# ishine/TargetDiarization

Measured on AMD Instinct MI355X. Metric: real-time factor (audio-sec/wall-sec) full infer() pipe, 16kHz mono, 1/2/4/8 GPU, higher is better.
Workload: dtype f32 (split-f16 x3: fp32-accurate products from three f16 MFMA passes, fp32 accumulate); 1 GPU; BASELINE configs[3]: 1800 s synthetic conversation (two alternating speakers, 20 % overlap) = 180 x 10 s windows: MossFormer2 (90 windows per launch) -> loudness swap -> ERes2NetV2 on every 10 s window of both streams + cosine vs a target embedding -> Paraformer (SANM encoder, CIF predictor, NAR decoder, argmax tokens + timestamps) on 30 s segments of both streams -> CT-Transformer punctuation of ; windows_per_launch=90

## Files before the change

targetdiarization_amd/csrc/eres2net.hip:

```cpp
#include <hip/hip_runtime.h>

#include <algorithm>
#include <cmath>
#include <string>
#include <vector>

#include "../../include/tdx.h"
#include "epilogues.hpp"
#include "weight_pack.hpp"
#include "weight_planes.hpp"

using namespace tdx;

namespace {

constexpr int NSTAGE = 4, SCALE = 4, EMB = 192;
const int kBlocks[NSTAGE] = {3, 4, 6, 3};
const int kPlanes[NSTAGE] = {64, 128, 256, 512};
const int kStride[NSTAGE] = {1, 2, 2, 2};

__global__ __launch_bounds__(256) void stem_kernel(const float* __restrict__ feat, const float* __restrict__ w9,
                                                    const float* __restrict__ bias, float* __restrict__ out, int F, long rows) {
    const long i = (long)blockIdx.x * 256 + threadIdx.x;
    if (i >= rows * 16) return;
// ... 73 lines not shown
struct EpiAffGate {
    const float* b; const float* x; long ldx; const float* y; long ldy; float* out; long ldo; int C;
    __device__ float col(int, int n) const { return b[n]; }
    __device__ EpiNone row(int, int) const { return EpiNone{}; }
    __device__ float2 aux(int, int m, int n, EpiNone) const {
        return n < C ? make_float2(x[(long)m * (int)ldx + n], y[(long)m * (int)ldy + n]) : make_float2(0.f, 0.f);
    }
    __device__ void store(int, int m, int n, float v, EpiNone, float c, float2 xy) const {
        if (n >= C) return;
        const float att = 1.0f + tanhf(v + c);
        out[(long)m * (int)ldo + n] = xy.x * att + xy.y * (2.0f - att);
    }
};


struct ChainX3Args {
    const float* in; long ldin;
    const unsigned char* wp; const float* ws; int wk;
    int cinp;
    const float* b;
    float* cat; long ldcat; int coff;
    const float* o1; long ldo1; int next_off; float* spin; int ldspin;
    int H, W;
};
template <int CIN, int TH>
struct ChainX3Cfg {
    static constexpr int KS = (CIN + 15) / 16, CP = KS * 16, PPB = CP * 4 + 16, NT = (CIN + 31) / 32, NB = NT * 32, MT = TH / 4;
    static constexpr int PATCH = (TH + 2) * 34 * PPB, BT = NB * PPB, LDS = PATCH + 2 * BT;
    static constexpr int BQ = NB * (CP / 8) * 2;
    static constexpr int BPT = (BQ + 255) / 256;
};
template <int CIN, int TH>
__global__ __launch_bounds__(256) void chain_conv_x3_kernel(ChainX3Args a) {
    using C = ChainX3Cfg<CIN, TH>;
    constexpr int KS = C::KS, CP = C::CP, PPB = C::PPB, NT = C::NT, MT = C::MT;
    static_assert(PPB % 32 == 16 && TH % 4 == 0 && CIN % 4 == 0, "pitch = odd multiple of 16 B");
    extern __shared__ __attribute__((aligned(16))) unsigned char lds[];
    unsigned char* const patch = lds;
    unsigned char* const bt = lds + C::PATCH;
    const int tid = threadIdx.x, lane = tid & 63, wave = tid >> 6, l31 = lane & 31, h = lane >> 5;
    const int x0 = blockIdx.x * 32, y0 = blockIdx.y * TH, b = blockIdx.z;
    typedef _Float16 h4 __attribute__((ext_vector_type(4)));
    typedef unsigned u32x4 __attribute__((ext_vector_type(4)));
    u32x4 breg[3][C::BPT];
#define TDX_CHAIN_BLOAD(tap_)                                                                                          \
    _Pragma("unroll") for (int i = 0; i < C::BPT; ++i) {                                                               \
// ... 95 lines not shown
    TDX_CHAIN_BSTORE(4) TDX_CHAIN_BLOAD(7) TDX_CHAIN_TAP(3) __syncthreads();
    TDX_CHAIN_BSTORE(5) TDX_CHAIN_BLOAD(8) TDX_CHAIN_TAP(4) __syncthreads();
    TDX_CHAIN_BSTORE(6) TDX_CHAIN_TAP(5) __syncthreads();
    TDX_CHAIN_BSTORE(7) TDX_CHAIN_TAP(6) __syncthreads();
    TDX_CHAIN_BSTORE(8) TDX_CHAIN_TAP(7) __syncthreads();
    TDX_CHAIN_TAP(8)
#undef TDX_CHAIN_TAP
#undef TDX_CHAIN_BSTORE
#undef TDX_CHAIN_BLOAD
#pragma unroll
    for (int n = 0; n < NT; ++n) {
        const int c = n * 32 + l31;
        const bool real = c < CIN;
#pragma unroll
        for (int m = 0; m < MT; ++m) {
            const int y = y0 + MT * wave + m;
            if (y >= a.H) continue;
#pragma unroll
            for (int i = 0; i < 16; ++i) {
                const int x = x0 + (i & 3) + 8 * (i >> 2) + 4 * h;
                if (x >= a.W) continue;
                const long mrow = ((long)b * a.H + y) * a.W + x;
                const float sp = relu20(acc[m][n][i] * sc[n] + bias[n]);
                if (real) a.cat[mrow * a.ldcat + a.coff + c] = sp;
                if (a.spin && c < a.ldspin) a.spin[mrow * a.ldspin + c] = real ? sp + nx[n][m][i] : 0.f;
            }
        }
    }
}
template <int CIN, int TH>
int launch_chain_x3(const ChainX3Args& a, int B, hipStream_t st) {
    using C = ChainX3Cfg<CIN, TH>;
    static const hipError_t attr_rc = hipFuncSetAttribute((const void*)chain_conv_x3_kernel<CIN, TH>, hipFuncAttributeMaxDynamicSharedMemorySize, C::LDS);
    if (attr_rc != hipSuccess) return tdx::fail_hip(attr_rc, __FILE__, __LINE__);
    hipLaunchKernelGGL((chain_conv_x3_kernel<CIN, TH>), dim3((a.W + 31) / 32, (a.H + TH - 1) / TH, B), dim3(256), C::LDS, st, a);
    LAUNCH_CHECK();
    return TDX_OK;
}

struct AffArgs {
    const float* x; long ldx; const float* y; long ldy;
    const float* w0; int ld0; const float* b0;
    const float* w3; int ld3; const float* b3;
    float* out; long ldo; long M;
};
template <int C>
struct AffCfg {
    static constexpr int IP = (C / 4 + 31) / 32 * 32, NT1 = IP / 32, NT2 = C / 32, NCH = 2 * C / 32;
    static constexpr int PA = 36, PT = IP + 4;
    static constexpr int AS = 128 * PA, WS = IP * PA;
    static constexpr int TS = 128 * PT;
    static constexpr int REG1 = (2 * AS > TS ? 2 * AS : TS);
    static constexpr int LDS = (REG1 + 2 * WS + C * PT) * 4;
    static constexpr int WPT = (IP * 8 + 255) / 256;
};
template <int C>
__global__ __launch_bounds__(256, C == 96 ? 2 : 1) void aff_fused_kernel(AffArgs a) {
    using F = AffCfg<C>;
    constexpr int IP = F::IP, NT1 = F::NT1, NT2 = F::NT2, NCH = F::NCH, PA = F::PA, PT = F::PT;
    extern __shared__ __attribute__((aligned(16))) float ldsf[];
    float* const As = ldsf;
    float* const Ws = ldsf + F::REG1;
    float* const W3s = Ws + 2 * F::WS;
    float* const Ts = ldsf;
    const int tid = threadIdx.x, lane = tid & 63, wave = tid >> 6, l31 = lane & 31, h = lane >> 5;
    const long m0 = (long)blockIdx.x * 128;
    f32x4 ra[4], rw[F::WPT];
// ... 78 lines not shown
                const f32x4 bv = *reinterpret_cast<const f32x4*>(Wb + n * 32 * PT + 8 * kk);
#pragma unroll
                for (int j = 0; j < 4; ++j) acc2[n] = __builtin_amdgcn_mfma_f32_32x32x2f32(av[j], bv[j], acc2[n], 0, 0, 0);
            }
        }
    }
#pragma unroll
    for (int n = 0; n < NT2; ++n) {
        const int c = n * 32 + l31;
        const float b3 = a.b3[c];
        float xv[16], yv[16];
#pragma unroll
        for (int r = 0; r < 16; ++r) {
            const long m = min(m0 + wave * 32 + (r & 3) + 8 * (r >> 2) + 4 * h, a.M - 1);
            xv[r] = a.x[m * a.ldx + c]; yv[r] = a.y[m * a.ldy + c];
        }
#pragma unroll
        for (int r = 0; r < 16; ++r) { tdx::touch(xv[r]); tdx::touch(yv[r]); }
#pragma unroll
        for (int r = 0; r < 16; ++r) {
            const long m = m0 + wave * 32 + (r & 3) + 8 * (r >> 2) + 4 * h;
            if (m >= a.M) continue;
            const float att = 1.0f + tanhf(acc2[n][r] + b3);
            a.out[m * a.ldo + c] = xv[r] * att + yv[r] * (2.0f - att);
        }
    }
}
template <int C>
int launch_aff_fused(const AffArgs& a, hipStream_t st) {
    using F = AffCfg<C>;
    static const hipError_t attr_rc = hipFuncSetAttribute((const void*)aff_fused_kernel<C>, hipFuncAttributeMaxDynamicSharedMemorySize, F::LDS);
    if (attr_rc != hipSuccess) return tdx::fail_hip(attr_rc, __FILE__, __LINE__);
    hipLaunchKernelGGL((aff_fused_kernel<C>), dim3((unsigned)((a.M + 127) / 128)), dim3(256), F::LDS, st, a);
    LAUNCH_CHECK();
    return TDX_OK;
}

__global__ __launch_bounds__(256) void split_rows_static_s2_kernel(const float* __restrict__ x, int ld, unsigned char* __restrict__ planes,
                                                                  long R, int K, int Hin, int Win, int Ho, int Wo, float s) {
    const long i = (long)blockIdx.x * 256 + threadIdx.x;
    const int per = K / 8;
    if (i >= R * per) return;
    const long row = i / per;
    const int ch = (int)(i - row * per);
    const long b = row / ((long)Ho * Wo);
    const int r = (int)(row - b * Ho * Wo), ho = r / Wo, wo = r - ho * Wo;
    const float* src = x + ((b * Hin + 2 * ho) * Win + 2 * wo) * ld + ch * 8;
// ... 47 lines not shown
    g.cv_Hin = Hin; g.cv_Win = Win; g.cv_Hout = Hout; g.cv_Wout = Wout; g.cv_stride = stride; g.cv_ntaps = tpb; g.cv_cin = cw.cinp;
    g.cv_taps_total = cw.taps;
    g.zero_row = zero_row;
    if (launch_gemm_h3x<false, false, false, false, EpiStoreZ, 0, true>(g, DS_SPLIT, EpiStoreZ{slab, (long)cw.Npad, M * cw.Npad}, st) != hipSuccess)
        return tdx::fail_hip(hipGetLastError(), __FILE__, __LINE__);
    const long MN = M * cw.Npad;
    hipLaunchKernelGGL(slab_reduce_kernel, dim3((unsigned)((MN / 4 + 255) / 256)), dim3(256), 0, st, slab, DS_SPLIT, MN, cw.Npad, bias, out);
    LAUNCH_CHECK();
    return TDX_OK;
}

}

struct tdx_eres2net {
    int device = 0;
    tdx::DevBuf dev; std::vector<BlockW> blocks; size_t stem_w, stem_b, seg_w, seg_b; ConvW ds; AffW fuse34;
    tdx::DevBuf dev_planes;
    size_t consts = 0;
};

namespace {

int run_aff(const tdx_eres2net* h, const AffW& a, const float* x, long ldx, const float* y, long ldy, float* tbuf, float* out, long ldo,
            long M, hipStream_t st) {
    if (a.C == 96 || a.C == 192) {
        AffArgs fa{x, ldx, y, ldy, h->dev + a.c0.w, a.c0.cinp, h->dev + a.c0.b, h->dev + a.c3.w, a.c3.cinp, h->dev + a.c3.b, out, ldo, M};
        return a.C == 96 ? launch_aff_fused<96>(fa, st) : launch_aff_fused<192>(fa, st);
    }
    {
        GemmSeg s0 = make_seg(x, ldx, h->dev + a.c0.w, 2L * a.C, a.C);
        GemmSeg s1 = make_seg(y, ldy, h->dev + a.c0.w + a.C, 2L * a.C, a.C);
        GemmArgs g = make_args((int)M, a.c0.Npad, s0);
        g.seg[1] = s1; g.nseg = 2;
        if (launch_gemm<false, false, false, false>(g, 1, EpiBiasActN<ActSilu>{h->dev + a.c0.b, tbuf, a.ipad, a.ipad}, st) != hipSuccess)
            return tdx::fail_hip(hipGetLastError(), __FILE__, __LINE__);
    }
    return linear_f32(tbuf, a.ipad, h->dev + a.c3.w, (int)M, a.c3.Npad, a.ipad, EpiAffGate{h->dev + a.c3.b, x, ldx, y, ldy, out, ldo, a.C}, st);
}

int run_aff34_x3(const tdx_eres2net* h, const AffW& a, const float* x, const float* y, float* tbuf, float* out, long M,
                 unsigned char* xP, unsigned char* yP, float* ys, unsigned char* tP, float* ts, const float* inv20, hipStream_t st) {
    const int C = a.C, IP = a.ipad;
    if (tdx::launch_h3_split_rows_static(x, C, xP, M, C, 1024.0f, st) != hipSuccess) return tdx::fail_hip(hipGetLastError(), __FILE__, __LINE__);
    if (tdx::launch_h3_split_rows(y, C, yP, ys, M, C, st) != hipSuccess) return tdx::fail_hip(hipGetLastError(), __FILE__, __LINE__);
    {
        H3Args g{};
        g.seg[0] = h3_seg(xP, inv20, 4L * C, a.c0.hp, a.c0.hs, 4L * 2 * C, C);
        g.seg[0].sa_mul = 0;
        g.seg[1] = h3_seg(yP, ys, 4L * C, a.c0.hp + 4L * C, a.c0.hs, 4L * 2 * C, C);
        g.nseg = 2; g.M = (int)M; g.N = a.c0.Npad;
        if (launch_gemm_h3x<false, false, false, true>(g, 1, EpiBiasActN<ActSilu>{h->dev + a.c0.b, tbuf, IP, IP}, st) != hipSuccess)
            return tdx::fail_hip(hipGetLastError(), __FILE__, __LINE__);
    }
    if (tdx::launch_h3_split_rows(tbuf, IP, tP, ts, M, IP, st) != hipSuccess) return tdx::fail_hip(hipGetLastError(), __FILE__, __LINE__);
    H3Args g{};
    g.seg[0] = h3_seg(tP, ts, 4L * IP, a.c3.hp, a.c3.hs, 4L * IP, IP);
    g.nseg = 1; g.M = (int)M; g.N = a.c3.Npad;
    if (launch_gemm_h3<false>(g, 1, EpiAffGate{h->dev + a.c3.b, x, (long)C, y, (long)C, out, (long)C, C}, st) != hipSuccess)
        return tdx::fail_hip(hipGetLastError(), __FILE__, __LINE__);
    return TDX_OK;
}

struct Dims { int H[5], W[5]; };
inline Dims make_dims(int F) {
    Dims d; d.H[0] = 80; d.W[0] = F;
    for (int s = 0; s < NSTAGE; ++s) {
        d.H[s + 1] = kStride[s] == 1 ? d.H[s] : (d.H[s] - 1) / 2 + 1;
        d.W[s + 1] = kStride[s] == 1 ? d.W[s] : (d.W[s] - 1) / 2 + 1;
    }
    return d;
}

}

extern "C" {

int tdx_eres2net_create(const void* blob, size_t blob_bytes, int device, tdx_eres2net** out) {
    if (!blob || !out) return tdx::fail(TDX_E_INVALID, "tdx_eres2net_create: null argument");
    tdx::Loader ld;
    if (!ld.parse(blob, blob_bytes)) return tdx::fail(TDX_E_BLOB, "tdx_eres2net_create: malformed TDXW blob");
    auto fold = [&](const std::string& wname, const std::string& bname, const std::string& bn, int N, int cin, int taps) -> ConvW {
        const float* W = ld.get(wname, (size_t)N * cin * taps);
        const float* cb = bname.empty() ? nullptr : ld.get(bname, N);
        const float *g = nullptr, *be = nullptr, *mu = nullptr, *var = nullptr;
// ... 131 lines not shown
    if (guard.err != hipSuccess) return tdx::fail_hip(guard.err, __FILE__, __LINE__);
    hipStream_t st = (hipStream_t)stream;
    const Dims d = make_dims(F);
    const size_t rows1 = (size_t)B * 80 * F;
    float* ws = (float*)ws_;
    float* P[3] = {ws, ws + wp.P, ws + 2 * wp.P};
    float* keep3 = ws + 3 * wp.P;
    float* o1 = keep3 + wp.keep3; float* cat = o1 + wp.o1;
    float* spin[2] = {cat + wp.o1, cat + wp.o1 + wp.spin};
    float* tbuf = spin[1] + wp.spin; float* stats = tbuf + wp.tbuf;
    unsigned char* hx = (unsigned char*)(stats + wp.stats);
    unsigned char* hcat = hx + wp.hx * sizeof(float);
    unsigned char* hin = hcat + wp.hcat * sizeof(float);
    float* slab = reinterpret_cast<float*>(hin + wp.hin * sizeof(float));
    const float* inv20 = h->dev + h->consts;
    const float* inv40 = h->dev + h->consts + 1;
    const unsigned char* zero_row = (const unsigned char*)(h->dev + h->consts + 64);

    hipLaunchKernelGGL(stem_kernel, dim3((unsigned)((rows1 * 16 + 255) / 256)), dim3(256), 0, st, feat, h->dev + h->stem_w, h->dev + h->stem_b, P[0], F, (long)rows1);
    LAUNCH_CHECK();
    const float* x = P[0];
    int cur = 0;
    int s = 0, cnt = 0;
    for (const BlockW& b : h->blocks) {
        const int Hin = (cnt == 0) ? d.H[s] : d.H[s + 1], Win = (cnt == 0) ? d.W[s] : d.W[s + 1];
        const int Ho = d.H[s + 1], Wo = d.W[s + 1];
        const long M = (long)B * Ho * Wo;
        const bool last_of_stage3 = (s == 2) && (cnt == kBlocks[2] - 1);
        const int iy = cur < 0 ? 0 : (cur + 1) % 3, ir = cur < 0 ? 1 : (cur + 2) % 3;
        float* y = last_of_stage3 ? keep3 : P[iy];
        float* res = P[ir];
        const bool x3 = b.conv1.hp != nullptr;
        const float* resid = x;
        if (x3) {
            int Hc = Hin, Wc = Win, sc_ = b.stride;
            if (b.stride == 2 && b.cin % 16 == 0) {
                const long R = (long)B * Ho * Wo;
                hipLaunchKernelGGL(split_rows_static_s2_kernel, dim3((unsigned)((R * (b.cin / 8) + 255) / 256)), dim3(256), 0, st,
                                   x, b.cin, hx, R, b.cin, Hin, Win, Ho, Wo, 1024.0f);
                LAUNCH_CHECK();
                Hc = Ho; Wc = Wo; sc_ = 1;
            } else if (tdx::launch_h3_split_rows_static(x, b.cin, hx, (long)B * Hin * Win, b.cin, 1024.0f, st) != hipSuccess)
                return tdx::fail_hip(hipGetLastError(), __FILE__, __LINE__);
            TRY(conv_gemm_h3(hx, inv20, zero_row, b.conv1, B, Hc, Wc, Ho, Wo, sc_, EpiBiasActN<ActRelu20>{h->dev + b.conv1.b, o1, b.w4, b.w4}, st));
            if (b.has_sc) {
                TRY(conv_gemm_h3(hx, inv20, zero_row, b.sc, B, Hc, Wc, Ho, Wo, sc_, EpiBiasActN<>{h->dev + b.sc.b, res, b.cout, b.cout}, st));
                resid = res;
            }
        } else {
            TRY(conv_gemm(x, b.cin, h->dev, b.conv1, B, Hin, Win, Ho, Wo, b.stride, EpiBiasActN<ActRelu20>{h->dev + b.conv1.b, o1, b.w4, b.w4}, st));
            if (b.has_sc) {
                TRY(conv_gemm(x, b.cin, h->dev, b.sc, B, Hin, Win, Ho, Wo, b.stride, EpiBiasActN<>{h->dev + b.sc.b, res, b.cout, b.cout}, st));
                resid = res;
            }
        }
        for (int j = 0; j < SCALE; ++j) {
            const float* in = j == 0 ? o1 : spin[j & 1];
            const long ldin = j == 0 ? b.w4 : b.wpad;
            const bool plain_next = (j + 1 < SCALE) && !b.is_aff;
            EpiChain e{h->dev + b.convs[j].b, cat, b.w4, j * b.width, b.width, b.wpad, o1, b.w4, (j + 1) * b.width,
                       plain_next ? spin[(j + 1) & 1] : nullptr};
            if (b.convs[j].hp && !b.is_aff && (b.width == 24 || b.width == 48)) {
                ChainX3Args ca{in, ldin, b.convs[j].hp, b.convs[j].hs, 9 * b.convs[j].cinp, b.convs[j].cinp, h->dev + b.convs[j].b, cat, b.w4, j * b.width,
                               o1, b.w4, (j + 1) * b.width, plain_next ? spin[(j + 1) & 1] : nullptr, b.wpad, Ho, Wo};
                if (b.width == 24) TRY((launch_chain_x3<24, 4>(ca, B, st)));
                else TRY((launch_chain_x3<48, 4>(ca, B, st)));
            } else if (x3) {
                if (tdx::launch_h3_split_rows_static(in, ldin, hin, M, b.wpad, 512.0f, st) != hipSuccess)
                    return tdx::fail_hip(hipGetLastError(), __FILE__, __LINE__);
                TRY(conv_gemm_h3(hin, inv40, zero_row, b.convs[j], B, Ho, Wo, Ho, Wo, 1, e, st));
            } else {
                TRY(conv_gemm(in, ldin, h->dev, b.convs[j], B, Ho, Wo, Ho, Wo, 1, e, st));
            }
            if (b.is_aff && j + 1 < SCALE)
                TRY(run_aff(h, b.aff[j], cat + j * b.width, b.w4, o1 + (j + 1) * b.width, b.w4, tbuf, spin[(j + 1) & 1], b.wpad, M, st));
        }
        if (x3) {
            if (tdx::launch_h3_split_rows_static(cat, b.w4, hcat, M, b.w4, 1024.0f, st) != hipSuccess)
                return tdx::fail_hip(hipGetLastError(), __FILE__, __LINE__);
            TRY(conv_gemm_h3(hcat, inv20, zero_row, b.conv3, B, Ho, Wo, Ho, Wo, 1, EpiBiasRes<ActRelu20>{h->dev + b.conv3.b, resid, y, b.cout}, st));
        } else {
            TRY(linear_f32(cat, b.w4, h->dev + b.conv3.w, (int)M, b.conv3.Npad, b.conv3.cinp, EpiBiasRes<ActRelu20>{h->dev + b.conv3.b, resid, y, b.cout}, st));
        }
        x = y;
        cur = last_of_stage3 ? -1 : iy;
        if (++cnt == kBlocks[s]) { cnt = 0; ++s; }
    }
    const int i_ds = (cur + 1) % 3, i_fu = (cur + 2) % 3;
    const long M4 = (long)B * d.H[4] * d.W[4];
    if (tdx::launch_h3_split_rows_static(keep3, 1024, hx, (long)B * d.H[3] * d.W[3], 1024, 1024.0f, st) != hipSuccess)
        return tdx::fail_hip(hipGetLastError(), __FILE__, __LINE__);
    if (wp.slab && h->ds.taps == 9 && h->ds.Npad == 2048)
        TRY(conv_gemm_h3_tapsplit(hx, inv20, zero_row, h->ds, B, d.H[3], d.W[3], d.H[4], d.W[4], 2, slab, nullptr, P[i_ds], st));
    else
        TRY(conv_gemm_h3(hx, inv20, zero_row, h->ds, B, d.H[3], d.W[3], d.H[4], d.W[4], 2, EpiBiasActN<>{nullptr, P[i_ds], 2048, 2048}, st));
    const char* aff34_env = getenv("TDX_ERES_AFF34_ROWS");
    const long aff34_min = aff34_env ? atol(aff34_env) : 8192;
    if (M4 >= aff34_min && 2 * M4 <= (long)B * 40960 && h->fuse34.c0.hp && h->fuse34.ipad == 512)
        TRY(run_aff34_x3(h, h->fuse34, x, P[i_ds], tbuf, P[i_fu], M4, hx, hcat, stats, hin, stats + M4, inv20, st));
    else
        TRY(run_aff(h, h->fuse34, x, 2048, P[i_ds], 2048, tbuf, P[i_fu], 2048, M4, st));
    hipLaunchKernelGGL(tstp_kernel, dim3(d.H[4], B), dim3(256), 0, st, P[i_fu], stats, d.W[4], 2048, d.H[4]);
    LAUNCH_CHECK();
    hipLaunchKernelGGL(seg_kernel, dim3(EMB, B), dim3(256), 0, st, stats, h->dev + h->seg_w, h->dev + h->seg_b, emb, 40960);
// ... 6 lines not shown
```

targetdiarization_amd/csrc/gemm_h3.hpp:

```cpp
#pragma once
#include <cstdio>
#include <cstdlib>
#include <typeinfo>
#include <vector>
#include <hip/hip_runtime.h>
#include <stdint.h>

#include "devutil.hpp"
#include "gemm.hpp"

namespace tdx {

typedef _Float16 f16x8 __attribute__((ext_vector_type(8)));

constexpr int H3_BM = 256, H3_BN = 256, H3_BK = 16, H3_THREADS = 512;
constexpr int H3_ROWB = 64;
constexpr int H3_OPER = 256 * H3_ROWB;
constexpr int H3_STAGE = 2 * H3_OPER;
constexpr int H3_NBUF = 4;
constexpr int H3_AUX_AHEAD = 3;
constexpr int H3_LDS = H3_NBUF * H3_STAGE;
constexpr int H3_LDS_EXTRA = 12288;

struct H3Seg {
// ... 221 lines not shown
    h4 a, b;
#pragma unroll
    for (int j = 0; j < 4; ++j) { const _Float16 t = (_Float16)xs[j]; a[j] = t; b[j] = (_Float16)(xs[j] - (float)t); }
    H3Pair r;
    r.hi = __builtin_bit_cast(uint2, a); r.lo = __builtin_bit_cast(uint2, b);
    return r;
}
__device__ __forceinline__ uint4 h3_pair16(int q, float4 v, float s) {
    const H3Pair o = h3_split4(v, s);
    const bool odd = q & 1;
    const uint2 send = odd ? o.hi : o.lo;
    uint2 recv;
    recv.x = (unsigned)__builtin_amdgcn_mov_dpp((int)send.x, 0xB1, 0xF, 0xF, true);
    recv.y = (unsigned)__builtin_amdgcn_mov_dpp((int)send.y, 0xB1, 0xF, 0xF, true);
    return odd ? make_uint4(recv.x, recv.y, o.lo.x, o.lo.y) : make_uint4(o.hi.x, o.hi.y, recv.x, recv.y);
}
__device__ __forceinline__ void h3_emit4(unsigned char* prow, int q, float4 v, float s) {
    *reinterpret_cast<uint4*>(prow + (q >> 1) * 32 + ((q & 1) ? 16 : 0)) = h3_pair16(q, v, s);
}
__device__ __forceinline__ void h3_emit4_pred(unsigned char* prow, int q, float4 v, float s, bool ok) {
    const uint4 w = h3_pair16(q, v, s);
    if (ok) *reinterpret_cast<uint4*>(prow + (q >> 1) * 32 + ((q & 1) ? 16 : 0)) = w;
}
__device__ __forceinline__ float h3_absmax4(float4 v) { return fmaxf(fmaxf(fabsf(v.x), fabsf(v.y)), fmaxf(fabsf(v.z), fabsf(v.w))); }


struct H3PlOut { unsigned char* planes; long pitch; float* scale; float* ss; long seg_stride; };
template <class E, class = void> struct epi_has_plout { static constexpr bool value = false; };
template <class E> struct epi_has_plout<E, decltype((void)&E::plout, void())> { static constexpr bool value = true; };
template <class E, class = void> struct epi_has_rowout { static constexpr bool value = false; };
template <class E> struct epi_has_rowout<E, decltype((void)&E::rowout, void())> { static constexpr bool value = true; };
struct H3Conv {
    const float* w; int wld;
    int ncols;
    unsigned char* planes; long pitch;
    float sv;
    float* u32; int u0; long ld32;
    int S, Sp;
};
template <class E, class = void> struct epi_has_conv { static constexpr bool value = false; };
template <class E> struct epi_has_conv<E, decltype((void)&E::conv, void())> { static constexpr bool value = true; };
constexpr int H3_CONV_STEP = 240, H3_CONV_HALO = 8;
template <class T> __device__ __forceinline__ void h3_assume_row(const T&) {}
__device__ __forceinline__ void h3_assume_row(long rw) { __builtin_assume(rw >= 0); }

template <bool A_TR, bool B_TR, bool PAIRED, bool TWOSEG, class Epi, int VARIANT = 0, bool A_CONV = false>
__global__ __launch_bounds__(H3_THREADS, 2) void gemm_h3_kernel(H3Args g, Epi epi) {
    static_assert(!A_CONV || (!A_TR && !TWOSEG), "A_CONV: row-major A planes, one weight segment");
    constexpr bool PINGPONG = VARIANT == 5;
    extern __shared__ __attribute__((aligned(1024))) unsigned char lds[];
    const int tid = threadIdx.x;
    const int lane = tid & 63, wave = tid >> 6;
    const int l31 = lane & 31, h = lane >> 5;
    const int wm = wave >> 2, wn = wave & 3;
// ... 590 lines not shown
            }
        } else {
            int nn[2];
            decltype(epi.col(0, 0)) cc[2];
            float sc[2];
#pragma unroll
            for (int tn = 0; tn < 2; ++tn) {
                nn[tn] = n0 + tn * 128 + lcol;
                cc[tn] = epi.col(z, nn[tn]);
                sc[tn] = sb[(long)nn[tn] * sbm];
            }
            touch(cc[0]); touch(cc[1]); touch(sc[0]); touch(sc[1]);
            unsigned char* const pbase = po.planes + (long)n0 * 4;
            auto phase2 = [&](int hf) {
                __syncthreads();
#pragma unroll 4
                for (int it = 0; it < 16; ++it) {
                    const int rl = wave * 16 + it;
                    const int lr = (rl >> 6) * 128 + (2 * hf + ((rl >> 5) & 1)) * 32 + (rl & 31);
                    const int m = m0 + lr;
                    const long pr = (!CHECK || m < g.M) ? epi.prow(z, min(m, g.M - 1)) : -1L;
                    const f32x4 v4 = *reinterpret_cast<const f32x4*>(T + rl * 256 + ((4 * lane) ^ (((rl >> 2) & 1) << 5)));
                    const float4 v = make_float4(v4[0], v4[1], v4[2], v4[3]);
                    const float mu = wave_max(h3_absmax4(v));
                    float q2 = (v.x * v.x + v.y * v.y) + (v.z * v.z + v.w * v.w);
                    if (po.ss) q2 = h3_wave_sum(q2);
                    float inv;
                    const float s_ = h3_row_scale(mu, inv);
                    if (pr >= 0) {
                        h3_emit4(pbase + pr * po.pitch, lane, v, s_);
                        if constexpr (epi_has_rowout<Epi>::value) *reinterpret_cast<f32x4*>(epi.rowout(z, pr, n0) + 4 * lane) = v4;
                        if (lane == 0) {
                            po.scale[(long)bn * po.seg_stride + pr] = inv;
                            if (po.ss) po.ss[(long)bn * po.seg_stride + pr] = q2;
                        }
                    }
                }
            };
            if constexpr (epi_has_aux<Epi>::value) {
                constexpr int AH = H3_AUX_AHEAD;
                decltype(epi.aux(0, 0, 0, RowT{})) ax[AH + 1][8];
                auto fetch = [&](int i, int set) {
                    const int tn = (i >> 2) & 1, tm = 2 * (i >> 3) + ((i >> 1) & 1), half = i & 1;
                    int lb = lrow + tm * 32;
                    asm volatile("" : "+v"(lb));
#pragma unroll
// ... 407 lines not shown
```

targetdiarization_amd/csrc/mf2.hip:

```cpp
#include <hip/hip_runtime.h>

#include <algorithm>
#include <cmath>
#include <cstdio>
#include <cstring>
#include <map>
#include <mutex>
#include <string>
#include <vector>

#include "../../include/tdx.h"
#include "gemm.hpp"
#include "gemm_x6.hpp"
#include "gemm_h3.hpp"
#include "gemm_h3a.hpp"
#include "mf2_kernels.hpp"
#include "mf2_attention.hpp"
#include "tdx_common.hpp"
#include "weight_planes.hpp"
#include "epilogues.hpp"

using namespace tdx;

namespace {
// ... 348 lines not shown
int ddn_core(const float* p, int B, int S, const float* w1T, const float* w2T, const float* ing, const float* inb,
             const float* pre, float* c1, float* c2, float* stat1, float* stat2, double* part, hipStream_t st) {
    const int ts = ddn_ts(B, S);
    const int nchunk1 = (S + ts - 1) / ts, nchunk2 = 2 * ((S + 2 * ts - 1) / (2 * ts));
    hipLaunchKernelGGL(ddn_conv1_kernel, dim3(nchunk1, B), dim3(256), 0, st, p, w1T, c1, part, S, nchunk1, ts);
    LAUNCH_CHECK();
    hipLaunchKernelGGL(in_finalize_kernel, dim3(B, 16), dim3(256), 0, st, part, stat1, nchunk1, S);
    LAUNCH_CHECK();
    hipLaunchKernelGGL(ddn_conv2_kernel, dim3(nchunk2, B), dim3(256), 0, st, c1, p, stat1, ing, inb, pre, w2T, c2, part, S, nchunk2, ts);
    LAUNCH_CHECK();
    hipLaunchKernelGGL(in_finalize_kernel, dim3(B, 16), dim3(256), 0, st, part, stat2, nchunk2, S);
    LAUNCH_CHECK();
    return TDX_OK;
}

template <class Epi>
int split_linear_h3(const float* A, long lda, unsigned char* hp, float* hs, int M, const H3W& W, int N, int K, Epi e, hipStream_t st) {
    if (tdx::launch_h3_split_rows(A, lda, hp, hs, M, K, st) != hipSuccess) return tdx::fail_hip(hipGetLastError(), __FILE__, __LINE__);
    return linear_h3(hp, hs, M, W, N, K, e, st);
}

inline bool fuse_conv() {
    static const bool on = [] { const char* e = getenv("TDX_FUSE_CONV"); return e ? atoi(e) != 0 : true; }();
    return on;
}
template <bool TWOSEG, class Epi>
hipError_t launch_linear_x3(tdx::H3Args g, Epi e, hipStream_t st) {
    return tdx::launch_gemm_h3x<false, false, false, TWOSEG>(g, 1, e, st);
}

}

extern "C" {

const char* tdx_version(void) { return "tdx 0.1.0 gfx950"; }
const char* tdx_last_error(void) { return tdx::last_error().c_str(); }

int tdx_mf2_create(const tdx_mf2_config* cfg, const void* blob, size_t blob_bytes, int device, tdx_mf2** out) {
    if (!cfg || !blob || !out) return tdx::fail(TDX_E_INVALID, "tdx_mf2_create: null argument");
    if (cfg->channels != C || cfg->num_spks != 2 || cfg->kernel_size != 16 || cfg->group_size != 256 || cfg->num_blocks < 1)
        return tdx::fail(TDX_E_INVALID, "tdx_mf2_create: unsupported config (need channels=512, spks=2, kernel=16, group=256)");
    tdx::Loader ld;
    if (!ld.parse(blob, blob_bytes)) return tdx::fail(TDX_E_BLOB, "tdx_mf2_create: malformed TDXW blob");
    const int L = cfg->num_blocks;
    ld.host.reserve(60u * 1000 * 1000);
    std::vector<float> stat_host((size_t)L * 2, 1.f);
// ... 331 lines not shown
        {
            tdx::H3Args g{};
            g.seg[0] = tdx::h3_seg(oP, os, 4L * 1024, w.hWo.p, w.hWo.s, 4L * 1024, 1024);
            g.seg[0].segk = 128; g.seg[0].strideSeg = M;
            g.nseg = 1; g.M = (int)M; g.N = C;
            EpiHiddenSN<8, false> e{oss, M, S, 0.03125f, w.go, w.bo, t, C};
            if (launch_linear_x3<false>(g, e, st) != hipSuccess) return tdx::fail_hip(hipGetLastError(), __FILE__, __LINE__);
        }
        {
            Conv17Args a{};
            a.in = t; a.ld_in = C; a.col0 = 0; a.wT = w.cw_o; a.C = C; a.out = x; a.ld_out = C; a.S = S; a.Sp = Sp; a.silu_in = 1;
            a.xp = xp; a.xs = xs; a.xs_stride = M;
            TRY(launch_conv17<1>(a, B, st));
        }
        if (h->taps && l == 0) hipMemcpyAsync(ws + P.tap0, x, M * C * sizeof(float), hipMemcpyDeviceToDevice, st);
        {
            tdx::H3Args g{};
            g.seg[0] = tdx::h3_seg(xp, xs, 4L * C, w.hW1.p, w.hW1.s, 4L * C, C);
            g.seg[0].segk = 256; g.seg[0].strideSeg = M;
            g.nseg = 1; g.M = (int)M; g.N = INNER;
            if (tdx::launch_gemm_h3x<false, false, false, false>(g, 1, EpiBiasPrelu{w.b1, w.a1, hraw, INNER}, st) != hipSuccess)
                return tdx::fail_hip(hipGetLastError(), __FILE__, __LINE__);
        }
        hipLaunchKernelGGL((layernorm_kernel<INNER, true>), rows4(M), dim3(256), 0, st, hraw, w.ln1g, w.ln1b, hh, (float*)nullptr, M, 1e-5f,
                           hp, hs);
        LAUNCH_CHECK();
        TRY(linear_h3(hp, hs, (int)M, w.hWuv, C, INNER, EpiBiasAct<ActSilu>{w.buv, uvpre, C}, st));
        {
            Conv17Args a{};
            a.in = uvpre; a.ld_in = C; a.col0 = 0; a.wT = w.cw_uv; a.C = C; a.out = uv; a.ld_out = C; a.S = S; a.Sp = Sp;
            a.xp = hp; a.xs = hs;
            TRY(launch_conv17<0>(a, B, st));
        }
        TRY(linear_h3(hp, hs, (int)M, w.hWl, INNER, INNER, EpiBiasReluPl{w.bl, fP, fs}, st));
        TRY(linear_h3(fP, fs, (int)M, w.hWp, INNER, INNER, EpiBiasAct<>{nullptr, p, INNER}, st));
        TRY(ddn_core(p, B, S, w.w1T, w.w2T, w.ing, w.inb, w.pre, c1, c2, stat1, stat2, part, st));
        hipLaunchKernelGGL(fsmn_tail_kernel, rows4(M), dim3(256), 0, st, c2, stat2, w.ing + INNER, w.inb + INNER, w.pre + INNER, uv, hh,
                           w.ln2g, w.ln2b, hp, hs, M, S);
        LAUNCH_CHECK();
        TRY(linear_h3(hp, hs, (int)M, w.hW2, C, INNER, EpiBiasResidualPl{w.b2, x, C, xp, xs, xss, M}, st));
        if (h->taps && l == 0) hipMemcpyAsync(ws + P.tap1, x, M * C * sizeof(float), hipMemcpyDeviceToDevice, st);
    }

    hipLaunchKernelGGL((layernorm_kernel<C, false>), rows4(M), dim3(256), 0, st, x, h->lnfg, h->lnfb, t, (float*)nullptr, M, 1e-6f);
    LAUNCH_CHECK();
    hipLaunchKernelGGL(rowblock_stats_kernel, dim3(P.nblk_gn, B), dim3(256), 0, st, t, part, S, 64, P.nblk_gn);
    LAUNCH_CHECK();
    hipLaunchKernelGGL(gn_finalize_kernel, dim3(B), dim3(64), 0, st, part, gnstat, P.nblk_gn, (double)S * C, 1e-8);
    LAUNCH_CHECK();
    float* r = uvpre;
    hipLaunchKernelGGL((gn_apply_kernel<1>), dim3((unsigned)((M * 128 + 255) / 256)), dim3(256), 0, st, t, gnstat, h->gn2g, h->gn2b, z,
                       h->prelu, r, M, S);
    LAUNCH_CHECK();
    float* r2 = o;
    TRY(split_linear_h3(r, C, hp, hs, (int)M, h->hWout, 2 * C, C, EpiBiasHalves{h->bout, r2, M}, st));
    float* gate = vu;
    {
        if (tdx::launch_h3_split_rows(r2, C, hp, hs, 2 * M, C, st) != hipSuccess) return tdx::fail_hip(hipGetLastError(), __FILE__, __LINE__);
        tdx::H3Args g{};
        g.seg[0] = tdx::h3_seg(hp, hs, 4L * C, h->hWtg.p, h->hWtg.s, 4L * C, C);
        g.seg[0].strideA = M * 4L * C; g.seg[0].strideSA = M;
// ... 125 lines not shown
```

targetdiarization_amd/csrc/mf2_kernels.hpp:

```cpp
#pragma once
#include <hip/hip_runtime.h>
#include <stdint.h>

#include "devutil.hpp"
#include "shared_kernels.hpp"

namespace tdx {

constexpr int ENC_TOK = 32;
__global__ __launch_bounds__(128) void encoder_kernel(const float* __restrict__ wav, const float* __restrict__ wT,
                                                       float* __restrict__ E, double* __restrict__ part, int T, int S,
                                                       int nblk) {
    __shared__ float seg[8 * ENC_TOK + 8];
    __shared__ double red[2][2];
    const int b = blockIdx.y, s0 = blockIdx.x * ENC_TOK, tid = threadIdx.x;
    const float* wv = wav + (long)b * T;
    for (int i = tid; i < 8 * ENC_TOK + 8; i += 128) {
        const int t = 8 * s0 + i;
        seg[i] = t < T ? wv[t] : 0.f;
    }
    float4 w[16];
#pragma unroll
    for (int t = 0; t < 16; ++t) w[t] = *reinterpret_cast<const float4*>(wT + t * 512 + tid * 4);
    __syncthreads();
// ... 306 lines not shown
#pragma unroll
        for (int i = 0; i < K - 1; ++i) win[i] = win[i + U];
    }
    part[(((long)b * nchunk2 + blockIdx.x) * 256 + j) * 2 + 0] = sum;
    part[(((long)b * nchunk2 + blockIdx.x) * 256 + j) * 2 + 1] = sq;
}

__global__ __launch_bounds__(256) void ddn_out_kernel(const float* __restrict__ c2, const float* __restrict__ stat2,
                                                       const float* __restrict__ in_g, const float* __restrict__ in_b,
                                                       const float* __restrict__ prelu, float* __restrict__ out, long M, int S) {
    const long i = (long)blockIdx.x * 256 + threadIdx.x;
    if (i >= M * 256) return;
    const int ch = (int)(i & 255);
    const int b = (int)((i >> 8) / S);
    float v = (c2[i] - stat2[(b * 256 + ch) * 2]) * stat2[(b * 256 + ch) * 2 + 1] * in_g[ch] + in_b[ch];
    out[i] = v >= 0.f ? v : prelu[ch] * v;
}

__global__ __launch_bounds__(256) void fsmn_tail_kernel(const float* __restrict__ c2, const float* __restrict__ stat2,
                                                         const float* __restrict__ in_g, const float* __restrict__ in_b,
                                                         const float* __restrict__ prelu, const float* __restrict__ uv,
                                                         const float* __restrict__ hh, const float* __restrict__ ln_g,
                                                         const float* __restrict__ ln_b, unsigned char* __restrict__ hp,
                                                         float* __restrict__ hs, long M, int S) {
    const long m = (long)blockIdx.x * 4 + (threadIdx.x >> 6);
    if (m >= M) return;
    const int lane = threadIdx.x & 63, c = lane * 4;
    const int b = (int)(m / S);
    const float4 cv = *reinterpret_cast<const float4*>(c2 + m * 256 + c);
    const float4 xu = *reinterpret_cast<const float4*>(uv + m * 512 + c);
    const float4 xv = *reinterpret_cast<const float4*>(uv + m * 512 + 256 + c);
    const float4 h4 = *reinterpret_cast<const float4*>(hh + m * 256 + c);
    const float* st = stat2 + (long)(b * 256 + c) * 2;
    const float4 ig = *reinterpret_cast<const float4*>(in_g + c);
    const float4 ib = *reinterpret_cast<const float4*>(in_b + c);
    const float4 al = *reinterpret_cast<const float4*>(prelu + c);
    float o[4] = {cv.x, cv.y, cv.z, cv.w};
    const float igv[4] = {ig.x, ig.y, ig.z, ig.w}, ibv[4] = {ib.x, ib.y, ib.z, ib.w}, alv[4] = {al.x, al.y, al.z, al.w};
    const float xuv[4] = {xu.x, xu.y, xu.z, xu.w}, xvv[4] = {xv.x, xv.y, xv.z, xv.w}, hv[4] = {h4.x, h4.y, h4.z, h4.w};
    float g[4];
    float s = 0.f;
#pragma unroll
    for (int i = 0; i < 4; ++i) {
        float v = (o[i] - st[i * 2]) * st[i * 2 + 1] * igv[i] + ibv[i];
        v = v >= 0.f ? v : alv[i] * v;
        g[i] = xvv[i] * (xuv[i] + v) + hv[i];
        s += g[i];
    }
    const float mean = wave_sum(s) * (1.0f / 256);
    float q = 0.f;
#pragma unroll
    for (int i = 0; i < 4; ++i) { g[i] -= mean; q = fmaf(g[i], g[i], q); }
    const float rstd = 1.0f / sqrtf(wave_sum(q) * (1.0f / 256) + 1e-5f);
    const float4 lg = *reinterpret_cast<const float4*>(ln_g + c);
    const float4 lb = *reinterpret_cast<const float4*>(ln_b + c);
// ... 186 lines not shown
```

targetdiarization_amd/csrc/shared_kernels.hpp:

```cpp
#pragma once
#include <hip/hip_runtime.h>
#include <stdint.h>

#include "devutil.hpp"
#include "gemm_h3.hpp"

namespace tdx {

template <int C, bool DUAL>
__global__ __launch_bounds__(256) void layernorm_kernel(const float* __restrict__ x, const float* __restrict__ g1,
                                                         const float* __restrict__ b1, float* __restrict__ out1,
                                                         float* __restrict__ out2, long M, float eps,
                                                         unsigned char* __restrict__ hp = nullptr, float* __restrict__ hs = nullptr) {
    constexpr int NV = C / 256;
    const long m = (long)blockIdx.x * 4 + (threadIdx.x >> 6);
    if (m >= M) return;
    const int lane = threadIdx.x & 63;
    float4 v[NV];
    float s = 0.f;
#pragma unroll
    for (int i = 0; i < NV; ++i) {
        v[i] = *reinterpret_cast<const float4*>(x + m * C + (i * 64 + lane) * 4);
        s += (v[i].x + v[i].y) + (v[i].z + v[i].w);
    }
    const float mean = wave_sum(s) * (1.0f / C);
    float q = 0.f;
#pragma unroll
    for (int i = 0; i < NV; ++i) {
        v[i].x -= mean; v[i].y -= mean; v[i].z -= mean; v[i].w -= mean;
        q += (v[i].x * v[i].x + v[i].y * v[i].y) + (v[i].z * v[i].z + v[i].w * v[i].w);
    }
    const float rstd = 1.0f / sqrtf(wave_sum(q) * (1.0f / C) + eps);
    float s2 = 0.f;
#pragma unroll
    for (int i = 0; i < NV; ++i) {
        const int c = (i * 64 + lane) * 4;
        const float4 g = *reinterpret_cast<const float4*>(g1 + c);
        const float4 b = *reinterpret_cast<const float4*>(b1 + c);
        v[i].x = v[i].x * rstd * g.x + b.x; v[i].y = v[i].y * rstd * g.y + b.y;
        v[i].z = v[i].z * rstd * g.z + b.z; v[i].w = v[i].w * rstd * g.w + b.w;
        *reinterpret_cast<float4*>(out1 + m * C + c) = v[i];
        s2 += (v[i].x + v[i].y) + (v[i].z + v[i].w);
    }
    if (DUAL) {
        const float mean2 = wave_sum(s2) * (1.0f / C);
        float q2 = 0.f;
#pragma unroll
        for (int i = 0; i < NV; ++i) {
            v[i].x -= mean2; v[i].y -= mean2; v[i].z -= mean2; v[i].w -= mean2;
            q2 += (v[i].x * v[i].x + v[i].y * v[i].y) + (v[i].z * v[i].z + v[i].w * v[i].w);
        }
        const float rstd2 = 1.0f / sqrtf(wave_sum(q2) * (1.0f / C) + eps);
        float mu = 0.f;
#pragma unroll
        for (int i = 0; i < NV; ++i) {
            v[i].x *= rstd2; v[i].y *= rstd2; v[i].z *= rstd2; v[i].w *= rstd2;
            if (hp) mu = fmaxf(mu, h3_absmax4(v[i]));
            else *reinterpret_cast<float4*>(out2 + m * C + (i * 64 + lane) * 4) = v[i];
        }
        if (hp) {
            float inv;
            const float sc = h3_row_scale(wave_max(mu), inv);
#pragma unroll
            for (int i = 0; i < NV; ++i) h3_emit4(hp + m * (4L * C), i * 64 + lane, v[i], sc);
// ... 191 lines not shown
```

Before: 506.0 audio-s/s.

## Emit split-f16 planes directly from ERes2Net epilogues and recompute FSMN LayerNorm

ERes2Net chain-conv, AFF and conv3 epilogues now write the split-f16 operand planes for the next GEMM directly, using a static scale. This skips separate split_rows passes over cat, spin and the next block's input. In MossFormer2 FSMN, the first LayerNorm output is no longer stored; the tail kernel recomputes it from hraw, trading a small amount of recomputation for one fewer round trip of activations through memory. Env switches keep the old paths available, but the defaults enable the new ones. The conv3 planes path also writes per-lane paired values via DPP, which is a layout risk.

```diff
diff --git a/targetdiarization_amd/csrc/eres2net.hip b/targetdiarization_amd/csrc/eres2net.hip
--- a/targetdiarization_amd/csrc/eres2net.hip
+++ b/targetdiarization_amd/csrc/eres2net.hip
@@ -119,6 +119,7 @@
     float* cat; long ldcat; int coff;
     const float* o1; long ldo1; int next_off; float* spin; int ldspin;
     int H, W;
+    unsigned char* hcat; long hpitch;
 };
 template <int CIN, int TH>
 struct ChainX3Cfg {
@@ -260,7 +261,10 @@
                 if (x >= a.W) continue;
                 const long mrow = ((long)b * a.H + y) * a.W + x;
                 const float sp = relu20(acc[m][n][i] * sc[n] + bias[n]);
-                if (real) a.cat[mrow * a.ldcat + a.coff + c] = sp;
+                if (real) {
+                    if (a.hcat) tdx::h3_emit1(a.hcat + mrow * a.hpitch, a.coff + c, sp, 1024.0f);
+                    else a.cat[mrow * a.ldcat + a.coff + c] = sp;
+                }
                 if (a.spin && c < a.ldspin) a.spin[mrow * a.ldspin + c] = real ? sp + nx[n][m][i] : 0.f;
             }
         }
@@ -281,6 +285,7 @@
     const float* w0; int ld0; const float* b0;
     const float* w3; int ld3; const float* b3;
     float* out; long ldo; long M;
+    unsigned char* hp; long hpitch;
 };
 template <int C>
 struct AffCfg {
@@ -405,7 +410,11 @@
             const long m = m0 + wave * 32 + (r & 3) + 8 * (r >> 2) + 4 * h;
             if (m >= a.M) continue;
             const float att = 1.0f + tanhf(acc2[n][r] + b3);
-            a.out[m * a.ldo + c] = xv[r] * att + yv[r] * (2.0f - att);
+            float px = xv[r] * att, py = yv[r] * (2.0f - att);
+            asm volatile("" : "+v"(px), "+v"(py));
+            const float o = px + py;
+            if (a.hp) tdx::h3_emit1(a.hp + m * a.hpitch, c, o, 512.0f);
+            else a.out[m * a.ldo + c] = o;
         }
     }
 }
@@ -499,11 +508,12 @@
 namespace {
 
 int run_aff(const tdx_eres2net* h, const AffW& a, const float* x, long ldx, const float* y, long ldy, float* tbuf, float* out, long ldo,
-            long M, hipStream_t st) {
+            long M, hipStream_t st, unsigned char* hp = nullptr) {
     if (a.C == 96 || a.C == 192) {
-        AffArgs fa{x, ldx, y, ldy, h->dev + a.c0.w, a.c0.cinp, h->dev + a.c0.b, h->dev + a.c3.w, a.c3.cinp, h->dev + a.c3.b, out, ldo, M};
+        AffArgs fa{x, ldx, y, ldy, h->dev + a.c0.w, a.c0.cinp, h->dev + a.c0.b, h->dev + a.c3.w, a.c3.cinp, h->dev + a.c3.b, out, ldo, M, hp, 4L * a.C};
         return a.C == 96 ? launch_aff_fused<96>(fa, st) : launch_aff_fused<192>(fa, st);
     }
+    if (hp) return tdx::fail(TDX_E_INVALID, "run_aff: planes output needs the fused launch (C = 96 / 192)");
     {
         GemmSeg s0 = make_seg(x, ldx, h->dev + a.c0.w, 2L * a.C, a.C);
         GemmSeg s1 = make_seg(y, ldy, h->dev + a.c0.w + a.C, 2L * a.C, a.C);
@@ -537,6 +547,23 @@
         return tdx::fail_hip(hipGetLastError(), __FILE__, __LINE__);
     return TDX_OK;
 }
+
+inline bool eres_split_passes() {
+    static const bool on = [] { const char* e = getenv("TDX_ERES_SPLIT_PASSES"); return e ? atoi(e) != 0 : false; }();
+    return on;
+}
+
+struct EpiConv3 {
+    const float* b; const float* res; float* out; long ld; unsigned char* hx;
+    __device__ float col(int, int n) const { return b[n]; }
+    __device__ EpiNone row(int, int) const { return EpiNone{}; }
+    __device__ float aux(int, int m, int n, EpiNone) const { return res[(long)m * (int)ld + n]; }
+    __device__ float val(int, int, int, float v, EpiNone, float c, float r) const { return ActRelu20::f((v + c) + r); }
+    __device__ float* rowout(int, long m, int n0) const { return out + m * ld + n0; }
+    __device__ tdx::H3PlOut plout(int) const { return tdx::H3PlOut{hx, 4 * ld, nullptr, nullptr, 0}; }
+    __device__ long prow(int, int m) const { return m; }
+    __device__ float plstatic() const { return 1024.0f; }
+};
 
 struct Dims { int H[5], W[5]; };
 inline Dims make_dims(int F) {
@@ -714,7 +741,10 @@
     const float* x = P[0];
     int cur = 0;
     int s = 0, cnt = 0;
-    for (const BlockW& b : h->blocks) {
+    const bool passes = eres_split_passes();
+    bool hx_ready = false;
+    for (size_t bi = 0; bi < h->blocks.size(); ++bi) {
+        const BlockW& b = h->blocks[bi];
         const int Hin = (cnt == 0) ? d.H[s] : d.H[s + 1], Win = (cnt == 0) ? d.W[s] : d.W[s + 1];
         const int Ho = d.H[s + 1], Wo = d.W[s + 1];
         const long M = (long)B * Ho * Wo;
@@ -732,7 +762,7 @@
                                    x, b.cin, hx, R, b.cin, Hin, Win, Ho, Wo, 1024.0f);
                 LAUNCH_CHECK();
                 Hc = Ho; Wc = Wo; sc_ = 1;
-            } else if (tdx::launch_h3_split_rows_static(x, b.cin, hx, (long)B * Hin * Win, b.cin, 1024.0f, st) != hipSuccess)
+            } else if (!hx_ready && tdx::launch_h3_split_rows_static(x, b.cin, hx, (long)B * Hin * Win, b.cin, 1024.0f, st) != hipSuccess)
                 return tdx::fail_hip(hipGetLastError(), __FILE__, __LINE__);
             TRY(conv_gemm_h3(hx, inv20, zero_row, b.conv1, B, Hc, Wc, Ho, Wo, sc_, EpiBiasActN<ActRelu20>{h->dev + b.conv1.b, o1, b.w4, b.w4}, st));
             if (b.has_sc) {
@@ -746,6 +776,8 @@
                 resid = res;
             }
         }
+        const bool aff_planes = !passes && x3 && b.is_aff && (b.width == 96 || b.width == 192) && b.wpad == b.width;
+        const bool cat_planes = !passes && x3 && !b.is_aff && b.width == 48 && b.convs[0].hp;
         for (int j = 0; j < SCALE; ++j) {
             const float* in = j == 0 ? o1 : spin[j & 1];
             const long ldin = j == 0 ? b.w4 : b.wpad;
@@ -754,24 +786,31 @@
                        plain_next ? spin[(j + 1) & 1] : nullptr};
             if (b.convs[j].hp && !b.is_aff && (b.width == 24 || b.width == 48)) {
                 ChainX3Args ca{in, ldin, b.convs[j].hp, b.convs[j].hs, 9 * b.convs[j].cinp, b.convs[j].cinp, h->dev + b.convs[j].b, cat, b.w4, j * b.width,
-                               o1, b.w4, (j + 1) * b.width, plain_next ? spin[(j + 1) & 1] : nullptr, b.wpad, Ho, Wo};
+                               o1, b.w4, (j + 1) * b.width, plain_next ? spin[(j + 1) & 1] : nullptr, b.wpad, Ho, Wo,
+                               cat_planes ? hcat : nullptr, 4L * b.w4};
                 if (b.width == 24) TRY((launch_chain_x3<24, 4>(ca, B, st)));
                 else TRY((launch_chain_x3<48, 4>(ca, B, st)));
             } else if (x3) {
-                if (tdx::launch_h3_split_rows_static(in, ldin, hin, M, b.wpad, 512.0f, st) != hipSuccess)
+                if (!(aff_planes && j >= 1) && tdx::launch_h3_split_rows_static(in, ldin, hin, M, b.wpad, 512.0f, st) != hipSuccess)
                     return tdx::fail_hip(hipGetLastError(), __FILE__, __LINE__);
                 TRY(conv_gemm_h3(hin, inv40, zero_row, b.convs[j], B, Ho, Wo, Ho, Wo, 1, e, st));
             } else {
                 TRY(conv_gemm(in, ldin, h->dev, b.convs[j], B, Ho, Wo, Ho, Wo, 1, e, st));
             }
             if (b.is_aff && j + 1 < SCALE)
-                TRY(run_aff(h, b.aff[j], cat + j * b.width, b.w4, o1 + (j + 1) * b.width, b.w4, tbuf, spin[(j + 1) & 1], b.wpad, M, st));
+                TRY(run_aff(h, b.aff[j], cat + j * b.width, b.w4, o1 + (j + 1) * b.width, b.w4, tbuf, spin[(j + 1) & 1], b.wpad, M, st, aff_planes ? hin : nullptr));
         }
         if (x3) {
-            if (tdx::launch_h3_split_rows_static(cat, b.w4, hcat, M, b.w4, 1024.0f, st) != hipSuccess)
+            if (!cat_planes && tdx::launch_h3_split_rows_static(cat, b.w4, hcat, M, b.w4, 1024.0f, st) != hipSuccess)
                 return tdx::fail_hip(hipGetLastError(), __FILE__, __LINE__);
-            TRY(conv_gemm_h3(hcat, inv20, zero_row, b.conv3, B, Ho, Wo, Ho, Wo, 1, EpiBiasRes<ActRelu20>{h->dev + b.conv3.b, resid, y, b.cout}, st));
+            const BlockW* nb = bi + 1 < h->blocks.size() ? &h->blocks[bi + 1] : nullptr;
+            hx_ready = !passes && nb && nb->conv1.hp && nb->stride == 1 && nb->cin == b.cout && b.conv3.Npad == b.cout && b.cout % 256 == 0;
+            if (hx_ready)
+                TRY(conv_gemm_h3(hcat, inv20, zero_row, b.conv3, B, Ho, Wo, Ho, Wo, 1, EpiConv3{h->dev + b.conv3.b, resid, y, b.cout, hx}, st));
+            else
+                TRY(conv_gemm_h3(hcat, inv20, zero_row, b.conv3, B, Ho, Wo, Ho, Wo, 1, EpiBiasRes<ActRelu20>{h->dev + b.conv3.b, resid, y, b.cout}, st));
         } else {
+            hx_ready = false;
             TRY(linear_f32(cat, b.w4, h->dev + b.conv3.w, (int)M, b.conv3.Npad, b.conv3.cinp, EpiBiasRes<ActRelu20>{h->dev + b.conv3.b, resid, y, b.cout}, st));
         }
         x = y;
diff --git a/targetdiarization_amd/csrc/gemm_h3.hpp b/targetdiarization_amd/csrc/gemm_h3.hpp
--- a/targetdiarization_amd/csrc/gemm_h3.hpp
+++ b/targetdiarization_amd/csrc/gemm_h3.hpp
@@ -267,6 +267,16 @@
     const uint4 w = h3_pair16(q, v, s);
     if (ok) *reinterpret_cast<uint4*>(prow + (q >> 1) * 32 + ((q & 1) ? 16 : 0)) = w;
 }
+__device__ __forceinline__ void h3_emit1(unsigned char* prow, int k, float x, float s) {
+    const float xs = x * s;
+    const _Float16 a = (_Float16)xs;
+    const _Float16 b = (_Float16)(xs - (float)a);
+    const unsigned hi = __builtin_bit_cast(unsigned short, a), lo = __builtin_bit_cast(unsigned short, b);
+    const bool odd = k & 1;
+    const unsigned recv = (unsigned)__builtin_amdgcn_mov_dpp((int)(odd ? hi : lo), 0xB1, 0xF, 0xF, true);
+    const unsigned w = odd ? (recv | (lo << 16)) : (hi | (recv << 16));
+    *reinterpret_cast<unsigned*>(prow + (k >> 3) * 32 + (odd ? 16 : 0) + ((k & 7) >> 1) * 4) = w;
+}
 __device__ __forceinline__ float h3_absmax4(float4 v) { return fmaxf(fmaxf(fabsf(v.x), fabsf(v.y)), fmaxf(fabsf(v.z), fabsf(v.w))); }
 
 
@@ -275,6 +285,8 @@
 template <class E> struct epi_has_plout<E, decltype((void)&E::plout, void())> { static constexpr bool value = true; };
 template <class E, class = void> struct epi_has_rowout { static constexpr bool value = false; };
 template <class E> struct epi_has_rowout<E, decltype((void)&E::rowout, void())> { static constexpr bool value = true; };
+template <class E, class = void> struct epi_has_plstatic { static constexpr bool value = false; };
+template <class E> struct epi_has_plstatic<E, decltype((void)&E::plstatic, void())> { static constexpr bool value = true; };
 struct H3Conv {
     const float* w; int wld;
     int ncols;
@@ -911,6 +923,13 @@
                     const long pr = (!CHECK || m < g.M) ? epi.prow(z, min(m, g.M - 1)) : -1L;
                     const f32x4 v4 = *reinterpret_cast<const f32x4*>(T + rl * 256 + ((4 * lane) ^ (((rl >> 2) & 1) << 5)));
                     const float4 v = make_float4(v4[0], v4[1], v4[2], v4[3]);
+                    if constexpr (epi_has_plstatic<Epi>::value) {
+                        if (pr >= 0) {
+                            h3_emit4(pbase + pr * po.pitch, lane, v, epi.plstatic());
+                            if constexpr (epi_has_rowout<Epi>::value) *reinterpret_cast<f32x4*>(epi.rowout(z, pr, n0) + 4 * lane) = v4;
+                        }
+                        continue;
+                    }
                     const float mu = wave_max(h3_absmax4(v));
                     float q2 = (v.x * v.x + v.y * v.y) + (v.z * v.z + v.w * v.w);
                     if (po.ss) q2 = h3_wave_sum(q2);
diff --git a/targetdiarization_amd/csrc/mf2.hip b/targetdiarization_amd/csrc/mf2.hip
--- a/targetdiarization_amd/csrc/mf2.hip
+++ b/targetdiarization_amd/csrc/mf2.hip
@@ -394,6 +394,10 @@
 
 inline bool fuse_conv() {
     static const bool on = [] { const char* e = getenv("TDX_FUSE_CONV"); return e ? atoi(e) != 0 : true; }();
+    return on;
+}
+inline bool fsmn_hh() {
+    static const bool on = [] { const char* e = getenv("TDX_FSMN_HH"); return e ? atoi(e) != 0 : false; }();
     return on;
 }
 template <bool TWOSEG, class Epi>
@@ -771,8 +775,8 @@
             if (tdx::launch_gemm_h3x<false, false, false, false>(g, 1, EpiBiasPrelu{w.b1, w.a1, hraw, INNER}, st) != hipSuccess)
                 return tdx::fail_hip(hipGetLastError(), __FILE__, __LINE__);
         }
-        hipLaunchKernelGGL((layernorm_kernel<INNER, true>), rows4(M), dim3(256), 0, st, hraw, w.ln1g, w.ln1b, hh, (float*)nullptr, M, 1e-5f,
-                           hp, hs);
+        hipLaunchKernelGGL((layernorm_kernel<INNER, true>), rows4(M), dim3(256), 0, st, hraw, w.ln1g, w.ln1b, fsmn_hh() ? hh : (float*)nullptr,
+                           (float*)nullptr, M, 1e-5f, hp, hs);
         LAUNCH_CHECK();
         TRY(linear_h3(hp, hs, (int)M, w.hWuv, C, INNER, EpiBiasAct<ActSilu>{w.buv, uvpre, C}, st));
         {
@@ -784,8 +788,8 @@
         TRY(linear_h3(hp, hs, (int)M, w.hWl, INNER, INNER, EpiBiasReluPl{w.bl, fP, fs}, st));
         TRY(linear_h3(fP, fs, (int)M, w.hWp, INNER, INNER, EpiBiasAct<>{nullptr, p, INNER}, st));
         TRY(ddn_core(p, B, S, w.w1T, w.w2T, w.ing, w.inb, w.pre, c1, c2, stat1, stat2, part, st));
-        hipLaunchKernelGGL(fsmn_tail_kernel, rows4(M), dim3(256), 0, st, c2, stat2, w.ing + INNER, w.inb + INNER, w.pre + INNER, uv, hh,
-                           w.ln2g, w.ln2b, hp, hs, M, S);
+        hipLaunchKernelGGL(fsmn_tail_kernel, rows4(M), dim3(256), 0, st, c2, stat2, w.ing + INNER, w.inb + INNER, w.pre + INNER, uv,
+                           fsmn_hh() ? hh : hraw, w.ln2g, w.ln2b, hp, hs, M, S, fsmn_hh() ? nullptr : w.ln1g, fsmn_hh() ? nullptr : w.ln1b);
         LAUNCH_CHECK();
         TRY(linear_h3(hp, hs, (int)M, w.hW2, C, INNER, EpiBiasResidualPl{w.b2, x, C, xp, xs, xss, M}, st));
         if (h->taps && l == 0) hipMemcpyAsync(ws + P.tap1, x, M * C * sizeof(float), hipMemcpyDeviceToDevice, st);
diff --git a/targetdiarization_amd/csrc/mf2_kernels.hpp b/targetdiarization_amd/csrc/mf2_kernels.hpp
--- a/targetdiarization_amd/csrc/mf2_kernels.hpp
+++ b/targetdiarization_amd/csrc/mf2_kernels.hpp
@@ -352,7 +352,8 @@
                                                          const float* __restrict__ prelu, const float* __restrict__ uv,
                                                          const float* __restrict__ hh, const float* __restrict__ ln_g,
                                                          const float* __restrict__ ln_b, unsigned char* __restrict__ hp,
-                                                         float* __restrict__ hs, long M, int S) {
+                                                         float* __restrict__ hs, long M, int S,
+                                                         const float* __restrict__ ln1_g = nullptr, const float* __restrict__ ln1_b = nullptr) {
     const long m = (long)blockIdx.x * 4 + (threadIdx.x >> 6);
     if (m >= M) return;
     const int lane = threadIdx.x & 63, c = lane * 4;
@@ -360,7 +361,17 @@
     const float4 cv = *reinterpret_cast<const float4*>(c2 + m * 256 + c);
     const float4 xu = *reinterpret_cast<const float4*>(uv + m * 512 + c);
     const float4 xv = *reinterpret_cast<const float4*>(uv + m * 512 + 256 + c);
-    const float4 h4 = *reinterpret_cast<const float4*>(hh + m * 256 + c);
+    float4 h4 = *reinterpret_cast<const float4*>(hh + m * 256 + c);
+    if (ln1_g) {
+        const float mean1 = wave_sum((h4.x + h4.y) + (h4.z + h4.w)) * (1.0f / 256);
+        h4.x -= mean1; h4.y -= mean1; h4.z -= mean1; h4.w -= mean1;
+        const float q1 = __builtin_fmaf(h4.y, h4.y, h4.x * h4.x) + __builtin_fmaf(h4.z, h4.z, h4.w * h4.w);
+        const float rstd1 = 1.0f / sqrtf(__builtin_fmaf(wave_sum(q1), 1.0f / 256, 1e-5f));
+        const float4 g1 = *reinterpret_cast<const float4*>(ln1_g + c);
+        const float4 b1 = *reinterpret_cast<const float4*>(ln1_b + c);
+        h4.x = __builtin_fmaf(h4.x * rstd1, g1.x, b1.x); h4.y = __builtin_fmaf(h4.y * rstd1, g1.y, b1.y);
+        h4.z = __builtin_fmaf(h4.z * rstd1, g1.z, b1.z); h4.w = __builtin_fmaf(h4.w * rstd1, g1.w, b1.w);
+    }
     const float* st = stat2 + (long)(b * 256 + c) * 2;
     const float4 ig = *reinterpret_cast<const float4*>(in_g + c);
     const float4 ib = *reinterpret_cast<const float4*>(in_b + c);
diff --git a/targetdiarization_amd/csrc/shared_kernels.hpp b/targetdiarization_amd/csrc/shared_kernels.hpp
--- a/targetdiarization_amd/csrc/shared_kernels.hpp
+++ b/targetdiarization_amd/csrc/shared_kernels.hpp
@@ -39,7 +39,7 @@
         const float4 b = *reinterpret_cast<const float4*>(b1 + c);
         v[i].x = v[i].x * rstd * g.x + b.x; v[i].y = v[i].y * rstd * g.y + b.y;
         v[i].z = v[i].z * rstd * g.z + b.z; v[i].w = v[i].w * rstd * g.w + b.w;
-        *reinterpret_cast<float4*>(out1 + m * C + c) = v[i];
+        if (!DUAL || out1) *reinterpret_cast<float4*>(out1 + m * C + c) = v[i];
         s2 += (v[i].x + v[i].y) + (v[i].z + v[i].w);
     }
     if (DUAL) {
```

Result: no change. 510.4 audio-s/s (median of 6 runs) (+0.9%).
